# second-state/qwen3_asr_rs

Hardware: NVIDIA H100
Metric: real-time factor (audio-sec/wall-sec) Qwen3-ASR-0.6B 30s clips (higher is better)
Workload: dtype f32 (bf16 weights, fp32-exact activations)

## Files before the change

### qwen3_asr_rs_b200/csrc/decode_batch.cu

```cuda
#include <algorithm>
#include "mega_common.cuh"

namespace asrb {

namespace megab {
using namespace mega;

static constexpr int MAXSPLIT = 32;
static constexpr int MAXROWS = 8;
static constexpr int ATT_SCRATCH = 4 * HD + NCONS_WARPS * 2 * HD + NCONS_WARPS * 4 + 8 + 8 + 2 * HD;

struct Params {
    const DecLayerW* layers;
    const bf16* lm_head;
    const bf16* embed;
    const float* final_norm;
    const float* rope_cos; const float* rope_sin;
    float eps;
    int L, H, QD, KVD, I, V, nkv;
    int nb;
    float* x;
    float* kcache; float* vcache; size_t cache_layer_stride, cache_seq_stride; int max_ctx;
    float* part_val; int* part_idx; int n_part;
    int* pos; int* done; int* next_id; int* ids_out; int* n_out; int max_new;
// ... 46 lines not shown
            const uint32_t xrow = xp + (uint32_t)sq * (H * 2) + (uint32_t)swz16(xc0 + 2 * ks + bhalf, sq & 7) * 16u;
            uint32_t b00, b01, b10, b11, b20, b21;
            ldsm_x4(xrow + (uint32_t)bpl * PSTR, b00, b01, b10, b11);
            ldsm_x2(xrow + 2u * PSTR, b20, b21);
            mma16816(acc[nt], a0, a1, a2, a3, b00, b01);
            mma16816(acc1[nt], a0, a1, a2, a3, b10, b11);
            mma16816(acc2[nt], a0, a1, a2, a3, b20, b21);
        }
    }
#pragma unroll
    for (int nt = 0; nt < NT; ++nt)
#pragma unroll
        for (int k = 0; k < 4; ++k) acc[nt][k] += acc1[nt][k] + acc2[nt][k];
}

static constexpr uint32_t SX_EMPTY = 0xFFFFFFFFu;
__device__ __forceinline__ void sx_store(uint32_t* p, float v) {
    uint32_t b = __float_as_uint(v);
    if (b == SX_EMPTY) b = 0x7FFFFFFFu;
    asm volatile("red.relaxed.gpu.global.and.b32 [%0], %1;" ::"l"(p), "r"(b) : "memory");
}
__device__ __forceinline__ uint4 sx_load4(const uint32_t* p) {
    uint4 v;
    asm volatile("ld.relaxed.gpu.global.v4.u32 {%0, %1, %2, %3}, [%4];" : "=r"(v.x), "=r"(v.y), "=r"(v.z), "=r"(v.w) : "l"(p) : "memory");
    return v;
}

__device__ __forceinline__ void head_norm_rope_b(const uint2* __restrict__ src, uint32_t tag, const float* __restrict__ nw,
                                                 float eps, const float* __restrict__ cs, const float* __restrict__ sn,
                                                 float* dst, int lane) {
    float v[4];
    ll_poll4(src + lane, 32, tag, v);
    const float ss = warp_sum(v[0] * v[0] + v[1] * v[1] + v[2] * v[2] + v[3] * v[3]);
    const float r = 1.0f / sqrtf(ss / 128.f + eps);
#pragma unroll
    for (int i = 0; i < 4; ++i) v[i] = (v[i] * r) * __ldg(nw + lane + 32 * i);
#pragma unroll
    for (int i = 0; i < 2; ++i) {
        const int d = lane + 32 * i;
        const float c = cs[d], s = sn[d];
        const float a = v[i], b = v[i + 2];
// ... 755 lines not shown
```

### qwen3_asr_rs_b200/csrc/decode_mega.cu

```cuda
#include "mega_common.cuh"

namespace asrb {

namespace mega {

struct Params {
    const DecLayerW* layers;
    const bf16* lm_head;
    const bf16* embed;
    const float* final_norm;
    const float* rope_cos; const float* rope_sin;
    float eps;
    int L, H, QD, KVD, I, V, nq, nkv, group;
    float* x;
    float* kcache; float* vcache; size_t cache_layer_stride; int max_ctx;
    int nsplit;
    float* part_val; int* part_idx;
    int* pos; int* done; int* next_id; int* ids_out; int* n_out; int max_new;
    unsigned* bar;
    uint2* qkv_ll; uint2* part_ll; uint2* attn_ll; uint2* x_ll; uint2* act_ll;
    long long* dbg;
};

static_assert(KV_KEYS * HD * 4 == SLOT_BYTES, "K / V tiles travel through the weight ring: one tile per slot");

template <int K>
__device__ __forceinline__ void load_xr(const float* xs, float (&xr)[K / 32], int lane) {
    const int sw = ((lane >> 2) & 1) * 4;
#pragma unroll
    for (int c = 0; c < K / 256; ++c) {
        const float4 a = *reinterpret_cast<const float4*>(xs + (c * 32 + lane) * 8 + sw);
        const float4 b = *reinterpret_cast<const float4*>(xs + (c * 32 + lane) * 8 + 4 - sw);
        xr[c * 8 + 0] = a.x; xr[c * 8 + 1] = a.y; xr[c * 8 + 2] = a.z; xr[c * 8 + 3] = a.w;
        xr[c * 8 + 4] = b.x; xr[c * 8 + 5] = b.y; xr[c * 8 + 6] = b.z; xr[c * 8 + 7] = b.w;
    }
// ... 94 lines not shown
}

__device__ __forceinline__ float warp_reduce8(const float (&a)[8], int lane) {
    const bool h16 = lane & 16, h8 = lane & 8, h4 = lane & 4;
    float k[4];
#pragma unroll
    for (int i = 0; i < 4; ++i) k[i] = (h16 ? a[4 + i] : a[i]) + __shfl_xor_sync(0xffffffffu, h16 ? a[i] : a[4 + i], 16);
    float m0 = (h8 ? k[2] : k[0]) + __shfl_xor_sync(0xffffffffu, h8 ? k[0] : k[2], 8);
    float m1 = (h8 ? k[3] : k[1]) + __shfl_xor_sync(0xffffffffu, h8 ? k[1] : k[3], 8);
    float v = (h4 ? m1 : m0) + __shfl_xor_sync(0xffffffffu, h4 ? m0 : m1, 4);
    v += __shfl_xor_sync(0xffffffffu, v, 2);
    v += __shfl_xor_sync(0xffffffffu, v, 1);
    return v;
}

enum { ME_STORE = 0, ME_RESID = 1, ME_SWIGLU = 2, ME_ARGMAX = 3 };

template <int K>
__device__ __forceinline__ void consume_ksplit(const Slice& s, const Ring& ring, uint32_t& q, const float* xs, uint2* out,
                                               uint32_t tag, float* xres, float* part) {
    const int tid = threadIdx.x, lane = tid & 31, warp = tid >> 5;
    constexpr int NU = K / 8;
    constexpr int J = (NU + NCONS - 1) / NCONS;
    uint32_t grp = 0;
    for (int r = s.r0; r < s.r1;) {
        const int rowsA = min(s.rpc, s.r1 - r);
        const uint32_t slotA = q % ring.nslot;
        mbar_wait(&ring.full[slotA], (q / ring.nslot) & 1);
        const bool pair = s.rpc < 8 && r + rowsA < s.r1;
        const int rowsB = pair ? min(s.rpc, s.r1 - r - rowsA) : 0;
        const uint32_t slotB = (q + 1) % ring.nslot;
        if (pair) mbar_wait(&ring.full[slotB], ((q + 1) / ring.nslot) & 1);
        const uint4* baseA = reinterpret_cast<const uint4*>(ring.slots + (size_t)slotA * SLOT_BYTES);
        const uint4* baseB = reinterpret_cast<const uint4*>(ring.slots + (size_t)slotB * SLOT_BYTES);
        const int R = rowsA + rowsB;
// ... 29 lines not shown
            }
            const float v = warp_reduce8(acc, lane);
            if (g0 + 8 >= R) {
                __syncwarp();
                if (lane == 0) { mbar_arrive(&ring.empty[slotA]); if (pair) mbar_arrive(&ring.empty[slotB]); }
            }
            float* pb = part + (grp & 1) * 64;
            if ((lane & 3) == 0) pb[warp * 8 + (lane >> 2)] = v;
            cons_sync();
            if (tid < ng) {
                float t = pb[tid];
#pragma unroll
                for (int w8 = 1; w8 < NCONS_WARPS; ++w8) t += pb[w8 * 8 + tid];
                const int row = r + g0 + tid;
                const float nv = xres[row - s.r0] + t; xres[row - s.r0] = nv;
                ll_store(out + row, nv, tag);
            }
        }
        r += R; q += pair ? 2 : 1;
    }
}

template <int K, int EPI>
__device__ __forceinline__ void consume_quad(const Slice& s, const Ring& ring, uint32_t& q, const float* xs, uint2* out,
                                             uint32_t tag, float& best_v, int& best_i,
                                             const float* norm_w, float norm_r, long long* fine) {
    const int lane = threadIdx.x & 31, warp = threadIdx.x >> 5;
    int fi = 0;
#define CF() do { if (fine && threadIdx.x == 0 && fi < 24) fine[fi++] = clock64(); } while (0)
    CF();
    constexpr int NU = K / 8;
    float xr[K / 32];
    if (norm_w) load_xr_norm<K>(xs, norm_w, norm_r, xr, lane);
    else load_xr<K>(xs, xr, lane);
    cons_sync();
    CF();
    const int j = lane >> 3;
    for (int r = s.r0; r < s.r1;) {
        const int rowsA = min(s.rpc, s.r1 - r);
        const uint32_t slotA = q % ring.nslot;
// ... 6 lines not shown
        const uint4* baseA = reinterpret_cast<const uint4*>(ring.slots + (size_t)slotA * SLOT_BYTES);
        const uint4* baseB = reinterpret_cast<const uint4*>(ring.slots + (size_t)slotB * SLOT_BYTES);
        const int R = rowsA + rowsB;
        for (int i0 = 4 * warp; i0 < R; i0 += 4 * NCONS_WARPS) {
            const int nv = min(4, R - i0);
            const uint4* rp[4];
#pragma unroll
            for (int i = 0; i < 4; ++i) {
                const int ri = i0 + (i < nv ? i : 0);
                rp[i] = ri < rowsA ? baseA + (size_t)ri * NU : baseB + (size_t)(ri - rowsA) * NU;
            }
            const float v = row_dot4<K>(rp[0], rp[1], rp[2], rp[3], xr, lane);
            const int row = r + i0 + j;
            if (EPI == ME_SWIGLU) {
                const float up = __shfl_xor_sync(0xffffffffu, v, 8);
                if ((lane & 15) == 0 && j < nv) ll_store(out + (row >> 1), silu(v) * up, tag);
            } else if (EPI == ME_STORE) {
                if ((lane & 7) == 0 && j < nv) ll_store(out + row, v, tag);
            } else {
                if ((lane & 7) == 0 && j < nv && v > best_v) { best_v = v; best_i = row; }
            }
        }
        CF();
        __syncwarp();
        if (lane == 0) { mbar_arrive(&ring.empty[slotA]); if (pair) mbar_arrive(&ring.empty[slotB]); }
        r += R; q += pair ? 2 : 1;
    }
    CF();
#undef CF
}

template <int K, int EPI>
__device__ __forceinline__ void consume(const Slice& s, const Ring& ring, uint32_t& q, const float* xs, uint2* out,
                                        uint32_t tag, float* xres, float& best_v, int& best_i,
                                        const float* norm_w = nullptr, float norm_r = 1.f, long long* fine = nullptr,
                                        float* part = nullptr) {
    if constexpr (EPI == ME_RESID) { consume_ksplit<K>(s, ring, q, xs, out, tag, xres, part); return; }
    else if constexpr (K <= 1024) { consume_quad<K, EPI>(s, ring, q, xs, out, tag, best_v, best_i, norm_w, norm_r, fine); return; }
    const int lane = threadIdx.x & 31, warp = threadIdx.x >> 5;
    int fi = 0;
#define CF() do { if (fine && threadIdx.x == 0 && fi < 24) fine[fi++] = clock64(); } while (0)
    CF();
    constexpr int RSTEP = (EPI == ME_SWIGLU) ? 2 : 1;
    constexpr bool XREG = K <= 2048;
    constexpr bool DUAL = XREG && K <= 1024;
    constexpr int KX = XREG ? K : 256;
    constexpr int UPW = (DUAL && EPI != ME_SWIGLU) ? 2 : 1;
    const int sub = lane >> 4;
    float xr[XREG ? K / 32 : 1];
    if (XREG) {
        if (norm_w) load_xr_norm<KX>(xs, norm_w, norm_r, reinterpret_cast<float (&)[KX / 32]>(xr), lane);
        else load_xr<KX>(xs, reinterpret_cast<float (&)[KX / 32]>(xr), lane);
        cons_sync();
// ... 11 lines not shown
        for (int ub = first * UPW; ub < units_here; ub += NCONS_WARPS * UPW) {
            if (EPI == ME_SWIGLU) {
                const int row = r + ub * 2;
                float v0, v1;
                if (DUAL) {
                    const float v = row_dot2<KX>(base + (size_t)(ub * 2) * (K / 8), base + (size_t)(ub * 2 + 1) * (K / 8),
                                                 reinterpret_cast<const float (&)[KX / 32]>(xr), lane);
                    v0 = v; v1 = __shfl_xor_sync(0xffffffffu, v, 16);
                } else if (XREG) {
                    v0 = row_dot<KX>(base + (size_t)(ub * 2) * (K / 8), reinterpret_cast<const float (&)[KX / 32]>(xr), lane);
                    v1 = row_dot<KX>(base + (size_t)(ub * 2 + 1) * (K / 8), reinterpret_cast<const float (&)[KX / 32]>(xr), lane);
                } else {
                    v0 = row_dot_smem<K>(base + (size_t)(ub * 2) * (K / 8), xs, lane);
                    v1 = row_dot_smem<K>(base + (size_t)(ub * 2 + 1) * (K / 8), xs, lane);
                }
                if (lane == 0) ll_store(out + (row >> 1), silu(v0) * v1, tag);
            } else {
                bool act; int row; float v0;
                if (DUAL) {
                    const bool two = ub + 1 < units_here;
                    v0 = row_dot2<KX>(base + (size_t)ub * (K / 8), base + (size_t)(two ? ub + 1 : ub) * (K / 8),
                                      reinterpret_cast<const float (&)[KX / 32]>(xr), lane);
                    act = ((lane & 15) == 0) && (sub == 0 || two);
                    row = r + ub + sub;
                } else {
                    if (XREG) v0 = row_dot<KX>(base + (size_t)ub * (K / 8), reinterpret_cast<const float (&)[KX / 32]>(xr), lane);
                    else v0 = row_dot_smem<K>(base + (size_t)ub * (K / 8), xs, lane);
                    act = lane == 0; row = r + ub;
                }
                if (EPI == ME_STORE) {
                    if (act) ll_store(out + row, v0, tag);
                } else if (EPI == ME_RESID) {
                    if (act) { const float nv = xres[row - s.r0] + v0; xres[row - s.r0] = nv; ll_store(out + row, nv, tag); }
                } else {
                    if (act && v0 > best_v) { best_v = v0; best_i = row; }
                }
            }
        }
        unit += (units_here + UPW - 1) / UPW * UPW;
        CF();
        __syncwarp();
        if (lane == 0) mbar_arrive(&ring.empty[slot]);
    }
    CF();
#undef CF
    if (!XREG) cons_sync();
}

__device__ __forceinline__ float norm_scale(float ss, int n, float eps, float* red) {
    const int tid = threadIdx.x;
    ss = warp_sum(ss);
    if ((tid & 31) == 0) red[tid >> 5] = ss;
    cons_sync();
    float tot = 0.f;
#pragma unroll
    for (int i = 0; i < NCONS_WARPS; ++i) tot += red[i];
    return 1.0f / sqrtf(tot / n + eps);
}

__device__ __forceinline__ void head_norm_rope(const uint2* __restrict__ src, uint32_t tag, const float* __restrict__ nw,
                                               float eps, const float* __restrict__ cs, const float* __restrict__ sn,
// ... 60 lines not shown
        asm volatile("fence.mbarrier_init.release.cluster;" ::: "memory");
    }
    const int pos = __ldcg(p.pos);
    {
        const uint2* src = reinterpret_cast<const uint2*>(p.layers);
        uint2* dst = reinterpret_cast<uint2*>(ltab);
        for (int i = tid; i < p.L * (int)(sizeof(DecLayerW) / 8); i += NTHREADS) dst[i] = src[i];
        if (tid < 64) ropes[tid] = p.rope_cos[(size_t)pos * 64 + tid];
        else if (tid < 128) ropes[tid] = p.rope_sin[(size_t)pos * 64 + tid - 64];
    }
    __syncthreads();

    const bool att_cta = (int)blockIdx.x < p.nkv * p.nsplit;
    const int att_g = blockIdx.x / p.nsplit, att_sp = blockIdx.x % p.nsplit, att_j0 = att_sp * KV_KEYS;
    const int n_old = att_cta ? max(0, min(pos - att_j0, KV_KEYS)) : 0;
    uint32_t q = 0;
    if (is_producer) {
        if (lane == 0) {
            const uint64_t pol = l2_evict_first_policy();
            auto issue = [&](const void* src, uint32_t bytes) __attribute__((always_inline)) {
                const uint32_t slot = q % NS, par = (q / NS) & 1;
                mbar_wait(&ring.empty[slot], par ^ 1);
                mbar_expect_tx(&ring.full[slot], bytes);
                bulk_g2s_hint(ring.slots + (size_t)slot * SLOT_BYTES, src, bytes, &ring.full[slot], pol);
                ++q;
            };
            auto issue_slice = [&](const Slice& s) __attribute__((always_inline)) {
                for (int r = s.r0; r < s.r1; r += s.rpc) issue(s.W + (size_t)r * s.K, (uint32_t)min(s.rpc, s.r1 - r) * s.K * 2);
            };
            const size_t kv_row = ((size_t)att_g * p.max_ctx + att_j0) * HD;
// ... 28 lines not shown
            issue_slice(make_slice(p.lm_head, p.V, H, 1));
        }
        return;
    }

    long long* dbg_row = nullptr; int dbg_i = 0;
    if (p.dbg && (blockIdx.x == 0 || blockIdx.x == gridDim.x - 1)) dbg_row = p.dbg + (blockIdx.x == 0 ? 0 : DBG_SLOTS);
    MEGA_MARK();
    const int half = HD / 2;
    const float* cs = ropes;
    const float* sn = ropes + half;
    const unsigned G = gridDim.x;
    float best_v = -INFINITY; int best_i = 0x7fffffff;
    const unsigned epoch = __ldcg(p.bar + 1);
    const uint32_t tag_base = (epoch & 0xffffffu) << 8;
    const Slice xsl = make_slice(nullptr, H, QD, 1);
    Slice sl_qkv = make_slice(nullptr, QD + 2 * p.KVD, H, 1), sl_o = make_slice(nullptr, H, QD, 1),
          sl_gu = make_slice(nullptr, 2 * I, H, 2), sl_dn = make_slice(nullptr, H, I, 1);
    for (int i = tid; i < xsl.r1 - xsl.r0; i += NCONS) xres[i] = __ldcg(p.x + xsl.r0 + i);

    for (int l = 0; l < p.L; ++l) {
        const DecLayerW w = ltab[l];
        const uint32_t tl = tag_base | ((uint32_t)l << 3);
        const float* pb = pbuf + (l & 1) * PARAM_FLOATS;
        mbar_wait(&p_full[l & 1], (l >> 1) & 1);
        float nr;
        {
            float ss = 0.f;
            if (l == 0) { for (int i = tid; i < H; i += NCONS) { const float v = __ldcg(p.x + i); xs[xs_swz(i)] = v; ss = fmaf(v, v, ss); } }
            else { MEGA_FINE(0); MEGA_FINE(1); ss = ll_gather(p.x_ll, H, (tag_base | ((uint32_t)(l - 1) << 3)) | PH_XD, xs); MEGA_FINE(2); }
            nr = norm_scale(ss, H, p.eps, red);
            MEGA_FINE(3);
        }
        consume<H, ME_STORE>(sl_qkv, ring, q, xs, p.qkv_ll, tl | PH_QKV, xres, best_v, best_i, pb, nr);
        MEGA_FINE(4);
        MEGA_GT(0);
        MEGA_MARK();
        {
            const int nloc = n_old;
            const int nact = min(p.nsplit, (pos + KV_KEYS - 1) / KV_KEYS);
            const bool merger = att_cta && att_sp == 0;
            if (nloc > 0) {
                const int g = att_g;
                float* qs = xs;
                float* kn = qs + p.group * HD;
                float* vn = kn + HD;
                float* sc = vn + HD;
                float* ml = sc + p.group * KV_KEYS;
                float* osum = ml + 8;
                float* wml = osum + NCONS_WARPS * 2 * HD;
                float* snew = wml + NCONS_WARPS * 4;
                const uint32_t ksl = q % ring.nslot, vsl = (q + 1) % ring.nslot;
                const float* Ks = reinterpret_cast<const float*>(ring.slots + (size_t)ksl * SLOT_BYTES);
                const float* Vs = reinterpret_cast<const float*>(ring.slots + (size_t)vsl * SLOT_BYTES);
                MEGA_FINE(24);
                cons_sync();
// ... 169 lines not shown
                            ok = __all_sync(0xffffffffu, (mv.y == tg) && (lv.y == tg) && round_ok(0));
                        } while (!ok);
                        MEGA_FINE(35);
                        const float m_l = lane < nact ? __uint_as_float(mv.x) : (lane == nact ? snew[hq] : -INFINITY);
                        const float l_l = lane < nact ? __uint_as_float(lv.x) : (lane == nact ? 1.f : 0.f);
                        const float M = warp_max(m_l);
                        const float f = expf(m_l - M);
                        const float Lsum = warp_sum(f * l_l);
                        float O = __shfl_sync(0xffffffffu, f, nact) * vn[d];
                        for (int u0 = 0; u0 < nact; u0 += RB) {
                            if (u0 > 0) { do { load_round(u0); ok = __all_sync(0xffffffffu, round_ok(u0)); } while (!ok); }
#pragma unroll
                            for (int u = 0; u < RB; ++u)
                                if (u0 + u < nact) O = fmaf(__shfl_sync(0xffffffffu, f, u0 + u), __uint_as_float(ov[u].x), O);
                        }
                        ll_store(p.attn_ll + (size_t)(g * p.group + hq) * HD + d, O / Lsum, tl | PH_ATTN);
                    }
                }
                MEGA_FINE(31);
                cons_sync();
            }
        }
        MEGA_MARK();
        MEGA_FINE(32);
        ll_gather(p.attn_ll, QD, tl | PH_ATTN, xs);
        MEGA_FINE(33);
        MEGA_GT(2);
        cons_sync();
        consume<QD, ME_RESID>(sl_o, ring, q, xs, p.x_ll, tl | PH_XO, xres, best_v, best_i, nullptr, 1.f, nullptr, part);
        MEGA_FINE(34);
        MEGA_MARK();
        cons_sync();
        {
            MEGA_FINE(8); MEGA_FINE(9);
            const float ss = ll_gather(p.x_ll, H, tl | PH_XO, xs); MEGA_FINE(10);
            nr = norm_scale(ss, H, p.eps, red); MEGA_FINE(11);
        }
        consume<H, ME_SWIGLU>(sl_gu, ring, q, xs, p.act_ll, tl | PH_ACT, xres, best_v, best_i, pb + H, nr, (dbg_row && l == 5) ? dbg_row + 440 : nullptr);
        MEGA_FINE(12);
        MEGA_FINE(13);
        MEGA_MARK();
        MEGA_FINE(16); MEGA_FINE(17);
        ll_gather(p.act_ll, I, tl | PH_ACT, xs); MEGA_FINE(18);
        cons_sync();
        consume<I, ME_RESID>(sl_dn, ring, q, xs, p.x_ll, tl | PH_XD, xres, best_v, best_i, nullptr, 1.f, nullptr, part);
        MEGA_FINE(19);
        MEGA_FINE(20);
        MEGA_MARK();
        cons_sync();
        if (lane == 0) mbar_arrive(&p_empty[l & 1]);
    }
    float nrf;
    {
        const float ss = ll_gather(p.x_ll, H, (tag_base | ((uint32_t)(p.L - 1) << 3)) | PH_XD, xs);
        mbar_wait(&p_full[p.L & 1], (p.L >> 1) & 1);
        nrf = norm_scale(ss, H, p.eps, red);
    }
    consume<H, ME_ARGMAX>(make_slice(p.lm_head, p.V, H, 1), ring, q, xs, nullptr, 0u, xres, best_v, best_i,
                          pbuf + (p.L & 1) * PARAM_FLOATS, nrf);
    MEGA_MARK();
#pragma unroll
    for (int o = 8; o <= 16; o <<= 1) {
        const float ov = __shfl_xor_sync(0xffffffffu, best_v, o); const int oi = __shfl_xor_sync(0xffffffffu, best_i, o);
        if (ov > best_v || (ov == best_v && oi < best_i)) { best_v = ov; best_i = oi; }
    }
    cons_sync();
    if (lane == 0) { red[warp] = best_v; ired[warp] = best_i; }
    cons_sync();
    int& is_last = ired[63];
    if (tid == 0) {
        float v = -INFINITY; int idx = 0x7fffffff;
        for (int wq = 0; wq < NCONS_WARPS; ++wq)
            if (red[wq] > v || (red[wq] == v && ired[wq] < idx)) { v = red[wq]; idx = ired[wq]; }
// ... 17 lines not shown
            if (ov > v || (ov == v && oi < idx)) { v = ov; idx = oi; }
        }
        if (lane == 0) { red[warp] = v; ired[warp] = idx; }
        cons_sync();
        int& tok_s = ired[62];
        if (tid == 0) {
            for (int wq = 1; wq < NCONS_WARPS; ++wq)
                if (red[wq] > v || (red[wq] == v && ired[wq] < idx)) { v = red[wq]; idx = ired[wq]; }
            int tok = idx;
            const int n = *p.n_out;
            if (tok == 151643 || tok == 151645 || n >= p.max_new) { *p.done = 1; *p.next_id = -1; tok = -1; }
            else { p.ids_out[n] = tok; *p.n_out = n + 1; *p.pos = pos + 1; *p.next_id = tok; }
            tok_s = tok;
            p.bar[0] = 0;
            p.bar[1] = p.bar[1] + 1;
        }
        cons_sync();
        const int tok = tok_s;
        if (tok >= 0) {
            const bf16* e = p.embed + (size_t)tok * H;
            for (int i = tid; i < H; i += NCONS) p.x[i] = __bfloat162float(e[i]);
        }
    }
}

}

static long long* g_last_dbg = nullptr;

static int mega_xs_floats(int I) { return std::max(I, mega::XS_MIN) + 64; }
// ... 14 lines not shown
    if (B < 1 || c.head_dim != 128) return false;
    const int group = c.num_attention_heads / c.num_key_value_heads;
    if (group + 2 > mega::NCONS_WARPS) return false;
    if ((size_t)(group * 128 + 256 + group * mega::KV_KEYS + 8 + mega::NCONS_WARPS * 2 * 128 + mega::NCONS_WARPS * 4 + 8) > (size_t)mega_xs_floats(c.intermediate_size)) return false;
    if (m.ctx->smem_optin < mega_smem_bytes(c.hidden_size, c.intermediate_size, mega_nslot(c))) return false;
    if ((c.hidden_size + m.ctx->sm_count - 1) / m.ctx->sm_count + 1 > mega::XRES_MAX) return false;
    if (c.num_hidden_layers > 32) return false;
    if ((max_ctx + mega::KV_KEYS - 1) / mega::KV_KEYS > mega::MAX_SPLITS) return false;
    if (((max_ctx + mega::KV_KEYS - 1) / mega::KV_KEYS) * c.num_key_value_heads > m.ctx->sm_count) return false;
    return dims_match<1024, 2048, 3072>(c) || dims_match<2048, 2048, 6144>(c) || dims_match<256, 512, 512>(c);
}

size_t decode_mega_part_floats(const Model& m) {
    const asrb_dims& c = m.d.c;
    const int group = c.num_attention_heads / c.num_key_value_heads;
    const size_t words = (size_t)m.d.qkv_dim + (size_t)m.ctx->sm_count * group * mega::PSTRIDE + m.d.q_dim + c.hidden_size +
                         c.intermediate_size + 64;
    return 2 * words + 64;
}

void launch_decode_step_mega(const Model& m, const DecodeBufs& b, int B, float* kcache, float* vcache,
                             size_t cache_layer_stride, size_t cache_seq_stride, int max_ctx, int ctx_now, const MegaBufs& mb,
                             cudaStream_t st, int64_t* launches) {
    ASRB_REQUIRE(decode_mega_supported(m, B, ctx_now), ASRB_ERR_STATE, "fused decode step not supported for this model/batch/context");
    ASRB_REQUIRE(m.d_dec_layers && mb.bar && mb.part, ASRB_ERR_STATE, "fused decode step buffers missing");
    const asrb_dims& c = m.d.c;
    const int G = m.ctx->sm_count;
    const int group = c.num_attention_heads / c.num_key_value_heads;
    const int nsplit = std::min(mega::MAX_SPLITS, std::min(G / c.num_key_value_heads, (max_ctx + mega::KV_KEYS - 1) / mega::KV_KEYS));
    const size_t smem = mega_smem_bytes(c.hidden_size, c.intermediate_size, mega_nslot(c));
    const void* fn = nullptr;
    if (dims_match<1024, 2048, 3072>(c)) fn = (const void*)mega::decode_step_kernel<1024, 2048, 3072, 6>;
    else if (dims_match<2048, 2048, 6144>(c)) fn = (const void*)mega::decode_step_kernel<2048, 2048, 6144, 5>;
    else fn = (const void*)mega::decode_step_kernel<256, 512, 512, 6>;
    ASRB_CUDA_CHECK(cudaFuncSetAttribute(fn, cudaFuncAttributeMaxDynamicSharedMemorySize, (int)smem));
    for (int sb = 0; sb < B; ++sb) {
        mega::Params p{};
        p.layers = m.d_dec_layers; p.lm_head = m.lm_head; p.embed = m.embed; p.final_norm = m.final_norm_sw;
        p.rope_cos = m.rope_cos; p.rope_sin = m.rope_sin; p.eps = (float)c.rms_norm_eps;
        p.L = c.num_hidden_layers; p.H = c.hidden_size; p.QD = m.d.q_dim; p.KVD = m.d.kv_dim; p.I = c.intermediate_size;
        p.V = c.vocab_size; p.nq = c.num_attention_heads; p.nkv = c.num_key_value_heads; p.group = group;
        p.x = b.x + (size_t)sb * c.hidden_size;
        p.kcache = kcache + (size_t)sb * cache_seq_stride; p.vcache = vcache + (size_t)sb * cache_seq_stride;
        p.cache_layer_stride = cache_layer_stride; p.max_ctx = max_ctx; p.nsplit = nsplit;
        p.part_val = b.part_val; p.part_idx = b.part_idx;
        p.pos = b.pos + sb; p.done = b.done + sb; p.next_id = b.next_id + sb;
        p.ids_out = b.ids_out + (size_t)sb * b.max_new; p.n_out = b.n_out + sb; p.max_new = b.max_new;
        p.bar = mb.bar;
        uint2* w = reinterpret_cast<uint2*>(mb.part);
        p.qkv_ll = w; w += m.d.qkv_dim;
        p.part_ll = w; w += (size_t)G * group * mega::PSTRIDE;
        p.attn_ll = w; w += m.d.q_dim;
        p.x_ll = w; w += c.hidden_size;
        p.act_ll = w; w += c.intermediate_size;
        p.dbg = mb.dbg;
        g_last_dbg = mb.dbg;
        if (mb.steps_issued && ++*mb.steps_issued >= 0xFFFF00u) {
            ASRB_CUDA_CHECK(cudaMemsetAsync(mb.part, 0, mb.part_bytes, st));
            const unsigned one = 1;
            ASRB_CUDA_CHECK(cudaMemcpyAsync(mb.bar + 1, &one, sizeof(one), cudaMemcpyHostToDevice, st));
            *mb.steps_issued = 1;
        }
        void* args[] = {(void*)&p};
        ASRB_CUDA_CHECK(cudaLaunchCooperativeKernel(fn, dim3(G), dim3(mega::NTHREADS), args, smem, st));
        if (launches) *launches += 1;
    }
}

int decode_mega_debug_timeline(long long* out, int cap) {
// ... 9 lines not shown
```

### qwen3_asr_rs_b200/csrc/internal.h

```cpp
#pragma once
#include <atomic>
#include <map>
#include <string>
#include <vector>
#include "../../include/asr_b200.h"
#include "common.cuh"

namespace asrb {

struct Dims {
    asrb_dims c;
    int enc_hd;
    int chunk_frames;
    int chunks_per_window;
    int conv_h[4];
    int conv_w[4];
    int tok_per_chunk;
    int cpad;
    int feat;
    int q_dim, kv_dim, qkv_dim;
    void derive();
};
void validate_dims(const asrb_dims& d);
inline int conv_out_len(int l) { return (l - 1) / 2 + 1; }
// ... 121 lines not shown
    float* attn;
    float* act;
    float* logits;
    float* part_val; int* part_idx; int n_part;
    int* pos;
    int* done;
    int* next_id;
    int* ids_out;
    int* n_out;
    int max_new;
};
void launch_decode_step_phases(const Model& m, const DecodeBufs& b, int B, float* kcache, float* vcache,
                               size_t cache_layer_stride, size_t cache_seq_stride, int max_ctx,
                               bool write_logits, cudaStream_t st, int64_t* launches);
struct MegaBufs { unsigned* bar = nullptr; float* part = nullptr; long long* dbg = nullptr; size_t part_bytes = 0; unsigned* steps_issued = nullptr;
                  uint32_t* sx = nullptr; size_t sx_bytes = 0; int* sx_nb = nullptr; };
size_t decode_mega_part_floats(const Model& m);
size_t decode_batch_part_floats(const Model& m);
size_t decode_batch_sx_bytes(const Model& m);
bool decode_batch_supported(const Model& m, int B, int ctx);
int decode_mega_dbg_slots();
void launch_greedy(const Model& m, const DecodeBufs& b, int B, cudaStream_t st, int64_t* launches);
void launch_lmhead_argmax(const Model& m, const float* x_rows, const int* d_row_idx, int B,
                          const DecodeBufs& b, bool write_logits, cudaStream_t st, int64_t* launches);

}
```

### qwen3_asr_rs_b200/csrc/mega_common.cuh

```cuda
#pragma once
#include "internal.h"

namespace asrb {
namespace mega {

static constexpr int NCONS_WARPS = 8;
static constexpr int NCONS = NCONS_WARPS * 32;
static constexpr int NTHREADS = NCONS + 32;
static constexpr int SLOT_BYTES = 32 * 1024;
static constexpr int NSLOT_MAX = 6;
static constexpr int KV_KEYS = 64;
static constexpr int XS_MIN = 3072;
static constexpr int XRES_MAX = 64;
static constexpr int MAX_LAYERS = 32;
static constexpr int HD = 128;
static constexpr int PSTRIDE = HD + 2;
static constexpr int DBG_SLOTS = 1024;
static constexpr int MAX_SPLITS = 18;

enum { PH_QKV = 1, PH_PART = 2, PH_ATTN = 3, PH_XO = 4, PH_ACT = 5, PH_XD = 6 };

__device__ __forceinline__ uint32_t smem_u32(const void* p) { return (uint32_t)__cvta_generic_to_shared(p); }
__device__ __forceinline__ void mbar_init(uint64_t* bar, uint32_t count) {
    asm volatile("mbarrier.init.shared::cta.b64 [%0], %1;" ::"r"(smem_u32(bar)), "r"(count));
}
__device__ __forceinline__ void mbar_expect_tx(uint64_t* bar, uint32_t bytes) {
    asm volatile("mbarrier.arrive.expect_tx.shared::cta.b64 _, [%0], %1;" ::"r"(smem_u32(bar)), "r"(bytes) : "memory");
}
__device__ __forceinline__ void mbar_arrive(uint64_t* bar) {
    asm volatile("mbarrier.arrive.shared::cta.b64 _, [%0];" ::"r"(smem_u32(bar)) : "memory");
}
__device__ __forceinline__ void mbar_wait(uint64_t* bar, uint32_t parity) {
    asm volatile(
        "{\n"
        ".reg .pred p;\n"
// ... 11 lines not shown
__device__ __forceinline__ uint64_t l2_evict_first_policy() {
    uint64_t pol;
    asm volatile("createpolicy.fractional.L2::evict_first.b64 %0, 1.0;" : "=l"(pol));
    return pol;
}
__device__ __forceinline__ void bulk_g2s_hint(void* dst, const void* src, uint32_t bytes, uint64_t* bar, uint64_t pol) {
    asm volatile("cp.async.bulk.shared::cluster.global.mbarrier::complete_tx::bytes.L2::cache_hint [%0], [%1], %2, [%3], %4;"
                 ::"r"(smem_u32(dst)), "l"(src), "r"(bytes), "r"(smem_u32(bar)), "l"(pol) : "memory");
}
__device__ __forceinline__ void cons_sync() { asm volatile("bar.sync 1, %0;" ::"n"(NCONS) : "memory"); }

__device__ __forceinline__ void ll_store(uint2* p, float v, uint32_t tag) {
    const unsigned long long val = ((unsigned long long)tag << 32) | (unsigned long long)__float_as_uint(v);
    asm volatile("red.relaxed.gpu.global.max.u64 [%0], %1;" ::"l"(p), "l"(val) : "memory");
}
__device__ __forceinline__ uint4 ll_load2(const uint2* p) {
    uint4 v;
    asm volatile("ld.relaxed.gpu.global.v4.u32 {%0, %1, %2, %3}, [%4];" : "=r"(v.x), "=r"(v.y), "=r"(v.z), "=r"(v.w) : "l"(p) : "memory");
    return v;
}
__device__ __forceinline__ float ll_poll1(const uint2* p, uint32_t tag) {
    uint2 v;
    do {
        asm volatile("ld.relaxed.gpu.global.v2.u32 {%0, %1}, [%2];" : "=r"(v.x), "=r"(v.y) : "l"(p) : "memory");
    } while (v.y != tag);
    return __uint_as_float(v.x);
}
__device__ __forceinline__ void ll_poll4(const uint2* p, int stride, uint32_t tag, float (&out)[4]) {
    uint2 v[4];
    bool ok;
    do {
#pragma unroll
        for (int i = 0; i < 4; ++i)
            asm volatile("ld.relaxed.gpu.global.v2.u32 {%0, %1}, [%2];" : "=r"(v[i].x), "=r"(v[i].y) : "l"(p + (size_t)i * stride) : "memory");
        ok = (v[0].y == tag) && (v[1].y == tag) && (v[2].y == tag) && (v[3].y == tag);
    } while (!ok);
#pragma unroll
    for (int i = 0; i < 4; ++i) out[i] = __uint_as_float(v[i].x);
}
__device__ __forceinline__ int xs_swz(int e) { const int k = e >> 2; return ((k ^ ((k >> 3) & 1)) << 2) | (e & 3); }
__device__ __forceinline__ float ll_gather(const uint2* buf, int n, uint32_t tag, float* xs) {
    float ss = 0.f;
    const int pairs = n >> 1;
    constexpr int U = 8;
    for (int i0 = threadIdx.x; i0 < pairs; i0 += U * NCONS) {
        uint4 v[U];
#pragma unroll
        for (int u = 0; u < U; ++u) v[u] = make_uint4(0u, 0u, 0u, 0u);
        bool ok;
        do {
            ok = true;
#pragma unroll
            for (int u = 0; u < U; ++u) {
                const int i = i0 + u * NCONS;
                if (i < pairs && !(v[u].y == tag && v[u].w == tag)) v[u] = ll_load2(buf + 2 * i);
            }
#pragma unroll
            for (int u = 0; u < U; ++u) {
                const int i = i0 + u * NCONS;
                if (i < pairs) ok = ok && (v[u].y == tag) && (v[u].w == tag);
            }
        } while (!ok);
#pragma unroll
        for (int u = 0; u < U; ++u) {
            const int i = i0 + u * NCONS;
            if (i < pairs) {
                const float a = __uint_as_float(v[u].x), b = __uint_as_float(v[u].z);
                *reinterpret_cast<float2*>(xs + xs_swz(2 * i)) = make_float2(a, b);
                ss = fmaf(a, a, ss); ss = fmaf(b, b, ss);
            }
        }
    }
    return ss;
}

struct Ring {
    uint8_t* slots; uint64_t* full; uint64_t* empty;
    uint32_t nslot;
};

struct Slice { const bf16* W; int K, r0, r1, rpc; };
__device__ __forceinline__ Slice make_slice(const bf16* W, int N, int K, int rstep) {
    Slice s; s.W = W; s.K = K;
    const unsigned units = (unsigned)(N / rstep);
    const int u0 = (int)((blockIdx.x * units) / gridDim.x), u1 = (int)(((blockIdx.x + 1) * units) / gridDim.x);
    s.r0 = u0 * rstep; s.r1 = u1 * rstep;
    s.rpc = SLOT_BYTES / (K * 2);
    s.rpc &= ~1;
    return s;
// ... 5 lines not shown
```

### qwen3_asr_rs_b200/csrc/session.cu

```cuda
#include <algorithm>
#include <cstring>
#include "internal.h"

namespace asrb {

void model_set_tensor(Model* m, const char* name, int dtype, const int64_t* shape, int ndim, const void* host);
void model_finalize(Model* m);
struct IngestState;
IngestState* ingest_state_new();
void ingest_state_free(IngestState* st);
void ingest_pcm(IngestState* st, cudaStream_t stream, const void* const* pcm, const int64_t* n_frames, const int32_t* channels,
                const int32_t* rate, const int32_t* format, int batch, float* d_samples, int64_t max_samples_per_utt,
                int64_t* n_out, int64_t* soff_out);

static const int kPromptHead[9] = {151644, 8948, 198, 151645, 198, 151644, 872, 198, 151669};
static const int kPromptTail[6] = {151670, 151645, 198, 151644, 77091, 198};
static const int kAudioPad = 151676;

struct Session {
    Model* m = nullptr;
    cudaStream_t st = nullptr;
    int max_batch = 0, max_lang = 0, max_new = 0;
    int64_t max_samples = 0, max_npad = 0;
    int maxF = 0, maxC = 0, maxT = 0, maxS = 0, max_ctx = 0;
// ... 145 lines not shown
            s->mega.sx_nb = &s->sx_nb;
            int maxwin = 0, maxpersist = 0;
            cudaDeviceGetAttribute(&maxwin, cudaDevAttrMaxAccessPolicyWindowSize, m->ctx->device);
            cudaDeviceGetAttribute(&maxpersist, cudaDevAttrMaxPersistingL2CacheSize, m->ctx->device);
            if (maxwin > 0 && maxpersist > 0) {
                const size_t want = std::min<size_t>({s->mega.sx_bytes, (size_t)maxwin, (size_t)maxpersist});
                if (cudaDeviceSetLimit(cudaLimitPersistingL2CacheSize, want) == cudaSuccess) {
                    cudaStreamAttrValue av{};
                    av.accessPolicyWindow.base_ptr = s->mega.sx; av.accessPolicyWindow.num_bytes = want;
                    av.accessPolicyWindow.hitRatio = 1.0f; av.accessPolicyWindow.hitProp = cudaAccessPropertyPersisting;
                    av.accessPolicyWindow.missProp = cudaAccessPropertyStreaming;
                    if (cudaStreamSetAttribute(s->st, cudaStreamAttributeAccessPolicyWindow, &av) != cudaSuccess) cudaGetLastError();
                } else cudaGetLastError();
            }
        }
        if (getenv("ASRB_MEGA_DEBUG")) s->mega.dbg = salloc<long long>(s, decode_mega_dbg_slots(), true);
        ASRB_CUDA_CHECK(cudaMallocHost(&s->h_done, Bm * sizeof(int)));
        ASRB_CUDA_CHECK(cudaMallocHost(&s->h_nout, Bm * sizeof(int)));
        ASRB_CUDA_CHECK(cudaMallocHost(&s->h_next, Bm * sizeof(int)));
        ASRB_CUDA_CHECK(cudaMallocHost(&s->h_ids, Bm * max_new * sizeof(int)));
        ASRB_CUDA_CHECK(cudaDeviceSynchronize());
    } catch (...) { delete s; throw; }
    return s;
}

void session_free(Session* s) { delete s; }

void session_mel(Session* s, const float* const* samples, const int64_t* n_samples, int batch, int64_t* n_frames_out) {
    ASRB_REQUIRE(batch >= 1 && batch <= s->max_batch, ASRB_ERR_INVALID, "batch exceeds session capacity");
    ASRB_CUDA_CHECK(cudaSetDevice(s->m->ctx->device));
// ... 410 lines not shown
```

Before: 292.9.

## Replace tagged LL exchange buffers with double-buffered sentinel slots in mega decode

The single-sequence megakernel now exchanges the residual, attention output and MLP activation between CTAs through per-layer, per-step double-buffered 32-bit slots. These slots are pre-filled with an all-ones sentinel and written with an atomic AND, replacing the 64-bit tagged LL stores. Readers poll 16-byte vectors until no word is empty, which halves the exchanged bytes and drops the tag compares. Each CTA re-arms its slice of the other parity buffer at step start, and a new step counter selects the parity. This adds re-arming work and a memory footprint of 2×L layer buffers.

Measured after the change: 301.9, median of 6. +3.1%, better.

```diff
diff --git a/qwen3_asr_rs_b200/csrc/decode_batch.cu b/qwen3_asr_rs_b200/csrc/decode_batch.cu
--- a/qwen3_asr_rs_b200/csrc/decode_batch.cu
+++ b/qwen3_asr_rs_b200/csrc/decode_batch.cu
@@ -84,17 +84,6 @@
         for (int k = 0; k < 4; ++k) acc[nt][k] += acc1[nt][k] + acc2[nt][k];
 }
 
-static constexpr uint32_t SX_EMPTY = 0xFFFFFFFFu;
-__device__ __forceinline__ void sx_store(uint32_t* p, float v) {
-    uint32_t b = __float_as_uint(v);
-    if (b == SX_EMPTY) b = 0x7FFFFFFFu;
-    asm volatile("red.relaxed.gpu.global.and.b32 [%0], %1;" ::"l"(p), "r"(b) : "memory");
-}
-__device__ __forceinline__ uint4 sx_load4(const uint32_t* p) {
-    uint4 v;
-    asm volatile("ld.relaxed.gpu.global.v4.u32 {%0, %1, %2, %3}, [%4];" : "=r"(v.x), "=r"(v.y), "=r"(v.z), "=r"(v.w) : "l"(p) : "memory");
-    return v;
-}
 
 __device__ __forceinline__ void head_norm_rope_b(const uint2* __restrict__ src, uint32_t tag, const float* __restrict__ nw,
                                                  float eps, const float* __restrict__ cs, const float* __restrict__ sn,
diff --git a/qwen3_asr_rs_b200/csrc/decode_mega.cu b/qwen3_asr_rs_b200/csrc/decode_mega.cu
--- a/qwen3_asr_rs_b200/csrc/decode_mega.cu
+++ b/qwen3_asr_rs_b200/csrc/decode_mega.cu
@@ -18,7 +18,8 @@
     float* part_val; int* part_idx;
     int* pos; int* done; int* next_id; int* ids_out; int* n_out; int max_new;
     unsigned* bar;
-    uint2* qkv_ll; uint2* part_ll; uint2* attn_ll; uint2* x_ll; uint2* act_ll;
+    uint2* qkv_ll; uint2* part_ll;
+    uint32_t* sx;
     long long* dbg;
 };
 
@@ -143,11 +144,11 @@
     return v;
 }
 
-enum { ME_STORE = 0, ME_RESID = 1, ME_SWIGLU = 2, ME_ARGMAX = 3 };
+enum { ME_STORE = 0, ME_SWIGLU = 1, ME_ARGMAX = 2 };
 
 template <int K>
-__device__ __forceinline__ void consume_ksplit(const Slice& s, const Ring& ring, uint32_t& q, const float* xs, uint2* out,
-                                               uint32_t tag, float* xres, float* part) {
+__device__ __forceinline__ void consume_ksplit(const Slice& s, const Ring& ring, uint32_t& q, const float* xs, uint32_t* out,
+                                               float* xres, float* part) {
     const int tid = threadIdx.x, lane = tid & 31, warp = tid >> 5;
     constexpr int NU = K / 8;
     constexpr int J = (NU + NCONS - 1) / NCONS;
@@ -207,7 +208,7 @@
                 for (int w8 = 1; w8 < NCONS_WARPS; ++w8) t += pb[w8 * 8 + tid];
                 const int row = r + g0 + tid;
                 const float nv = xres[row - s.r0] + t; xres[row - s.r0] = nv;
-                ll_store(out + row, nv, tag);
+                sx_store(out + row, nv);
             }
         }
         r += R; q += pair ? 2 : 1;
@@ -216,7 +217,7 @@
 
 template <int K, int EPI>
 __device__ __forceinline__ void consume_quad(const Slice& s, const Ring& ring, uint32_t& q, const float* xs, uint2* out,
-                                             uint32_t tag, float& best_v, int& best_i,
+                                             uint32_t tag, uint32_t* sxo, float& best_v, int& best_i,
                                              const float* norm_w, float norm_r, long long* fine) {
     const int lane = threadIdx.x & 31, warp = threadIdx.x >> 5;
     int fi = 0;
@@ -253,7 +254,7 @@
             const int row = r + i0 + j;
             if (EPI == ME_SWIGLU) {
                 const float up = __shfl_xor_sync(0xffffffffu, v, 8);
-                if ((lane & 15) == 0 && j < nv) ll_store(out + (row >> 1), silu(v) * up, tag);
+                if ((lane & 15) == 0 && j < nv) sx_store(sxo + (row >> 1), silu(v) * up);
             } else if (EPI == ME_STORE) {
                 if ((lane & 7) == 0 && j < nv) ll_store(out + row, v, tag);
             } else {
@@ -271,11 +272,9 @@
 
 template <int K, int EPI>
 __device__ __forceinline__ void consume(const Slice& s, const Ring& ring, uint32_t& q, const float* xs, uint2* out,
-                                        uint32_t tag, float* xres, float& best_v, int& best_i,
-                                        const float* norm_w = nullptr, float norm_r = 1.f, long long* fine = nullptr,
-                                        float* part = nullptr) {
-    if constexpr (EPI == ME_RESID) { consume_ksplit<K>(s, ring, q, xs, out, tag, xres, part); return; }
-    else if constexpr (K <= 1024) { consume_quad<K, EPI>(s, ring, q, xs, out, tag, best_v, best_i, norm_w, norm_r, fine); return; }
+                                        uint32_t tag, uint32_t* sxo, float& best_v, int& best_i,
+                                        const float* norm_w = nullptr, float norm_r = 1.f, long long* fine = nullptr) {
+    if constexpr (K <= 1024) { consume_quad<K, EPI>(s, ring, q, xs, out, tag, sxo, best_v, best_i, norm_w, norm_r, fine); return; }
     const int lane = threadIdx.x & 31, warp = threadIdx.x >> 5;
     int fi = 0;
 #define CF() do { if (fine && threadIdx.x == 0 && fi < 24) fine[fi++] = clock64(); } while (0)
@@ -317,7 +316,7 @@
                     v0 = row_dot_smem<K>(base + (size_t)(ub * 2) * (K / 8), xs, lane);
                     v1 = row_dot_smem<K>(base + (size_t)(ub * 2 + 1) * (K / 8), xs, lane);
                 }
-                if (lane == 0) ll_store(out + (row >> 1), silu(v0) * v1, tag);
+                if (lane == 0) sx_store(sxo + (row >> 1), silu(v0) * v1);
             } else {
                 bool act; int row; float v0;
                 if (DUAL) {
@@ -333,8 +332,6 @@
                 }
                 if (EPI == ME_STORE) {
                     if (act) ll_store(out + row, v0, tag);
-                } else if (EPI == ME_RESID) {
-                    if (act) { const float nv = xres[row - s.r0] + v0; xres[row - s.r0] = nv; ll_store(out + row, nv, tag); }
                 } else {
                     if (act && v0 > best_v) { best_v = v0; best_i = row; }
                 }
@@ -348,6 +345,50 @@
     CF();
 #undef CF
     if (!XREG) cons_sync();
+}
+
+template <int N>
+__device__ __forceinline__ float sx_gather(const uint32_t* src, float* xs) {
+    const int tid = threadIdx.x, lane = tid & 31, warp = tid >> 5;
+    constexpr int NQ = N / 4;
+    constexpr int KQ = (NQ + NCONS - 1) / NCONS;
+    int qi[KQ];
+    uint4 v[KQ];
+#pragma unroll
+    for (int k = 0; k < KQ; ++k) {
+        qi[k] = 16 * warp + (lane & 15) + (NCONS / 2) * (2 * k + (lane >> 4));
+        v[k] = make_uint4(SX_EMPTY, SX_EMPTY, SX_EMPTY, SX_EMPTY);
+    }
+    bool ok;
+    do {
+        ok = true;
+#pragma unroll
+        for (int k = 0; k < KQ; ++k)
+            if (qi[k] < NQ && !sx_ready(v[k])) v[k] = sx_load4(src + 4 * qi[k]);
+#pragma unroll
+        for (int k = 0; k < KQ; ++k)
+            if (qi[k] < NQ) ok = ok && sx_ready(v[k]);
+    } while (!ok);
+#pragma unroll
+    for (int k = 0; k < KQ; ++k)
+        if (qi[k] < NQ) *reinterpret_cast<uint4*>(xs + xs_swz(4 * qi[k])) = v[k];
+    __syncwarp();
+    float ss = 0.f;
+#pragma unroll
+    for (int i = tid; i < N / 2; i += NCONS) {
+        const float2 x = *reinterpret_cast<const float2*>(xs + xs_swz(2 * i));
+        ss = fmaf(x.x, x.x, ss); ss = fmaf(x.y, x.y, ss);
+    }
+    return ss;
+}
+
+template <int N>
+__device__ __forceinline__ void sx_copy(const uint32_t* src, float* xs) {
+    for (int j = threadIdx.x; j < N / 4; j += NCONS) {
+        uint4 v;
+        do { v = sx_load4(src + 4 * j); } while (!sx_ready(v));
+        *reinterpret_cast<uint4*>(xs + xs_swz(4 * j)) = v;
+    }
 }
 
 __device__ __forceinline__ float norm_scale(float ss, int n, float eps, float* red) {
@@ -438,6 +479,20 @@
     const bool att_cta = (int)blockIdx.x < p.nkv * p.nsplit;
     const int att_g = blockIdx.x / p.nsplit, att_sp = blockIdx.x % p.nsplit, att_j0 = att_sp * KV_KEYS;
     const int n_old = att_cta ? max(0, min(pos - att_j0, KV_KEYS)) : 0;
+    const bool merger = att_cta && att_sp == 0;
+    const Slice xsl = make_slice(nullptr, H, QD, 1), sl_gu = make_slice(nullptr, 2 * I, H, 2);
+
+    constexpr size_t SXL = 2 * H + QD + I;
+    const unsigned sstep = __ldcg(p.bar + 3);
+    uint32_t* const sx_cur = p.sx + (size_t)(sstep & 1u) * p.L * SXL;
+    auto rearm = [&](int l) __attribute__((always_inline)) {
+        uint32_t* const base = p.sx + (size_t)((sstep & 1u) ^ 1u) * p.L * SXL + (size_t)l * SXL;
+        const int xrows = xsl.r1 - xsl.r0, a0 = sl_gu.r0 / 2, arows = sl_gu.r1 / 2 - a0;
+        const int nattn = merger ? p.group * HD : 0;
+        for (int i = tid; i < xrows; i += NCONS) { base[xsl.r0 + i] = SX_EMPTY; base[H + xsl.r0 + i] = SX_EMPTY; }
+        for (int i = tid; i < nattn; i += NCONS) base[2 * H + att_g * p.group * HD + i] = SX_EMPTY;
+        for (int i = tid; i < arows; i += NCONS) base[2 * H + QD + a0 + i] = SX_EMPTY;
+    };
     uint32_t q = 0;
     if (is_producer) {
         if (lane == 0) {
@@ -496,32 +551,34 @@
     float best_v = -INFINITY; int best_i = 0x7fffffff;
     const unsigned epoch = __ldcg(p.bar + 1);
     const uint32_t tag_base = (epoch & 0xffffffu) << 8;
-    const Slice xsl = make_slice(nullptr, H, QD, 1);
-    Slice sl_qkv = make_slice(nullptr, QD + 2 * p.KVD, H, 1), sl_o = make_slice(nullptr, H, QD, 1),
-          sl_gu = make_slice(nullptr, 2 * I, H, 2), sl_dn = make_slice(nullptr, H, I, 1);
+    Slice sl_qkv = make_slice(nullptr, QD + 2 * p.KVD, H, 1), sl_o = make_slice(nullptr, H, QD, 1), sl_dn = make_slice(nullptr, H, I, 1);
     for (int i = tid; i < xsl.r1 - xsl.r0; i += NCONS) xres[i] = __ldcg(p.x + xsl.r0 + i);
+    for (int l = 0; l < p.L; ++l) rearm(l);
 
     for (int l = 0; l < p.L; ++l) {
         const DecLayerW w = ltab[l];
         const uint32_t tl = tag_base | ((uint32_t)l << 3);
         const float* pb = pbuf + (l & 1) * PARAM_FLOATS;
+        uint32_t* const sx_xo = sx_cur + (size_t)l * SXL;
+        uint32_t* const sx_xd = sx_xo + H;
+        uint32_t* const sx_attn = sx_xo + 2 * H;
+        uint32_t* const sx_act = sx_xo + 2 * H + QD;
         mbar_wait(&p_full[l & 1], (l >> 1) & 1);
         float nr;
         {
             float ss = 0.f;
             if (l == 0) { for (int i = tid; i < H; i += NCONS) { const float v = __ldcg(p.x + i); xs[xs_swz(i)] = v; ss = fmaf(v, v, ss); } }
-            else { MEGA_FINE(0); MEGA_FINE(1); ss = ll_gather(p.x_ll, H, (tag_base | ((uint32_t)(l - 1) << 3)) | PH_XD, xs); MEGA_FINE(2); }
+            else { MEGA_FINE(0); MEGA_FINE(1); ss = sx_gather<H>(sx_xd - SXL, xs); MEGA_FINE(2); }
             nr = norm_scale(ss, H, p.eps, red);
             MEGA_FINE(3);
         }
-        consume<H, ME_STORE>(sl_qkv, ring, q, xs, p.qkv_ll, tl | PH_QKV, xres, best_v, best_i, pb, nr);
+        consume<H, ME_STORE>(sl_qkv, ring, q, xs, p.qkv_ll, tl | PH_QKV, nullptr, best_v, best_i, pb, nr);
         MEGA_FINE(4);
         MEGA_GT(0);
         MEGA_MARK();
         {
             const int nloc = n_old;
             const int nact = min(p.nsplit, (pos + KV_KEYS - 1) / KV_KEYS);
-            const bool merger = att_cta && att_sp == 0;
             if (nloc > 0) {
                 const int g = att_g;
                 float* qs = xs;
@@ -721,7 +778,7 @@
                             for (int u = 0; u < RB; ++u)
                                 if (u0 + u < nact) O = fmaf(__shfl_sync(0xffffffffu, f, u0 + u), __uint_as_float(ov[u].x), O);
                         }
-                        ll_store(p.attn_ll + (size_t)(g * p.group + hq) * HD + d, O / Lsum, tl | PH_ATTN);
+                        sx_store(sx_attn + (size_t)(g * p.group + hq) * HD + d, O / Lsum);
                     }
                 }
                 MEGA_FINE(31);
@@ -730,27 +787,27 @@
         }
         MEGA_MARK();
         MEGA_FINE(32);
-        ll_gather(p.attn_ll, QD, tl | PH_ATTN, xs);
+        sx_copy<QD>(sx_attn, xs);
         MEGA_FINE(33);
         MEGA_GT(2);
         cons_sync();
-        consume<QD, ME_RESID>(sl_o, ring, q, xs, p.x_ll, tl | PH_XO, xres, best_v, best_i, nullptr, 1.f, nullptr, part);
+        consume_ksplit<QD>(sl_o, ring, q, xs, sx_xo, xres, part);
         MEGA_FINE(34);
         MEGA_MARK();
         cons_sync();
         {
             MEGA_FINE(8); MEGA_FINE(9);
-            const float ss = ll_gather(p.x_ll, H, tl | PH_XO, xs); MEGA_FINE(10);
+            const float ss = sx_gather<H>(sx_xo, xs); MEGA_FINE(10);
             nr = norm_scale(ss, H, p.eps, red); MEGA_FINE(11);
         }
-        consume<H, ME_SWIGLU>(sl_gu, ring, q, xs, p.act_ll, tl | PH_ACT, xres, best_v, best_i, pb + H, nr, (dbg_row && l == 5) ? dbg_row + 440 : nullptr);
+        consume<H, ME_SWIGLU>(sl_gu, ring, q, xs, nullptr, 0u, sx_act, best_v, best_i, pb + H, nr, (dbg_row && l == 5) ? dbg_row + 440 : nullptr);
         MEGA_FINE(12);
         MEGA_FINE(13);
         MEGA_MARK();
         MEGA_FINE(16); MEGA_FINE(17);
-        ll_gather(p.act_ll, I, tl | PH_ACT, xs); MEGA_FINE(18);
+        sx_copy<I>(sx_act, xs); MEGA_FINE(18);
         cons_sync();
-        consume<I, ME_RESID>(sl_dn, ring, q, xs, p.x_ll, tl | PH_XD, xres, best_v, best_i, nullptr, 1.f, nullptr, part);
+        consume_ksplit<I>(sl_dn, ring, q, xs, sx_xd, xres, part);
         MEGA_FINE(19);
         MEGA_FINE(20);
         MEGA_MARK();
@@ -759,11 +816,11 @@
     }
     float nrf;
     {
-        const float ss = ll_gather(p.x_ll, H, (tag_base | ((uint32_t)(p.L - 1) << 3)) | PH_XD, xs);
+        const float ss = sx_gather<H>(sx_cur + (size_t)(p.L - 1) * SXL + H, xs);
         mbar_wait(&p_full[p.L & 1], (p.L >> 1) & 1);
         nrf = norm_scale(ss, H, p.eps, red);
     }
-    consume<H, ME_ARGMAX>(make_slice(p.lm_head, p.V, H, 1), ring, q, xs, nullptr, 0u, xres, best_v, best_i,
+    consume<H, ME_ARGMAX>(make_slice(p.lm_head, p.V, H, 1), ring, q, xs, nullptr, 0u, nullptr, best_v, best_i,
                           pbuf + (p.L & 1) * PARAM_FLOATS, nrf);
     MEGA_MARK();
 #pragma unroll
@@ -811,6 +868,7 @@
             tok_s = tok;
             p.bar[0] = 0;
             p.bar[1] = p.bar[1] + 1;
+            p.bar[3] = p.bar[3] + 1;
         }
         cons_sync();
         const int tok = tok_s;
@@ -855,16 +913,19 @@
 size_t decode_mega_part_floats(const Model& m) {
     const asrb_dims& c = m.d.c;
     const int group = c.num_attention_heads / c.num_key_value_heads;
-    const size_t words = (size_t)m.d.qkv_dim + (size_t)m.ctx->sm_count * group * mega::PSTRIDE + m.d.q_dim + c.hidden_size +
-                         c.intermediate_size + 64;
+    const size_t words = (size_t)m.d.qkv_dim + (size_t)m.ctx->sm_count * group * mega::PSTRIDE + 64;
     return 2 * words + 64;
+}
+size_t decode_mega_sx_bytes(const Model& m) {
+    const asrb_dims& c = m.d.c;
+    return 2 * (size_t)c.num_hidden_layers * (2 * (size_t)c.hidden_size + m.d.q_dim + c.intermediate_size) * sizeof(uint32_t);
 }
 
 void launch_decode_step_mega(const Model& m, const DecodeBufs& b, int B, float* kcache, float* vcache,
                              size_t cache_layer_stride, size_t cache_seq_stride, int max_ctx, int ctx_now, const MegaBufs& mb,
                              cudaStream_t st, int64_t* launches) {
     ASRB_REQUIRE(decode_mega_supported(m, B, ctx_now), ASRB_ERR_STATE, "fused decode step not supported for this model/batch/context");
-    ASRB_REQUIRE(m.d_dec_layers && mb.bar && mb.part, ASRB_ERR_STATE, "fused decode step buffers missing");
+    ASRB_REQUIRE(m.d_dec_layers && mb.bar && mb.part && mb.sx_seq, ASRB_ERR_STATE, "fused decode step buffers missing");
     const asrb_dims& c = m.d.c;
     const int G = m.ctx->sm_count;
     const int group = c.num_attention_heads / c.num_key_value_heads;
@@ -890,10 +951,8 @@
         p.bar = mb.bar;
         uint2* w = reinterpret_cast<uint2*>(mb.part);
         p.qkv_ll = w; w += m.d.qkv_dim;
-        p.part_ll = w; w += (size_t)G * group * mega::PSTRIDE;
-        p.attn_ll = w; w += m.d.q_dim;
-        p.x_ll = w; w += c.hidden_size;
-        p.act_ll = w; w += c.intermediate_size;
+        p.part_ll = w;
+        p.sx = mb.sx_seq;
         p.dbg = mb.dbg;
         g_last_dbg = mb.dbg;
         if (mb.steps_issued && ++*mb.steps_issued >= 0xFFFF00u) {
diff --git a/qwen3_asr_rs_b200/csrc/internal.h b/qwen3_asr_rs_b200/csrc/internal.h
--- a/qwen3_asr_rs_b200/csrc/internal.h
+++ b/qwen3_asr_rs_b200/csrc/internal.h
@@ -159,8 +159,10 @@
                                size_t cache_layer_stride, size_t cache_seq_stride, int max_ctx,
                                bool write_logits, cudaStream_t st, int64_t* launches);
 struct MegaBufs { unsigned* bar = nullptr; float* part = nullptr; long long* dbg = nullptr; size_t part_bytes = 0; unsigned* steps_issued = nullptr;
-                  uint32_t* sx = nullptr; size_t sx_bytes = 0; int* sx_nb = nullptr; };
+                  uint32_t* sx = nullptr; size_t sx_bytes = 0; int* sx_nb = nullptr;
+                  uint32_t* sx_seq = nullptr; };
 size_t decode_mega_part_floats(const Model& m);
+size_t decode_mega_sx_bytes(const Model& m);
 size_t decode_batch_part_floats(const Model& m);
 size_t decode_batch_sx_bytes(const Model& m);
 bool decode_batch_supported(const Model& m, int B, int ctx);
diff --git a/qwen3_asr_rs_b200/csrc/mega_common.cuh b/qwen3_asr_rs_b200/csrc/mega_common.cuh
--- a/qwen3_asr_rs_b200/csrc/mega_common.cuh
+++ b/qwen3_asr_rs_b200/csrc/mega_common.cuh
@@ -18,7 +18,7 @@
 static constexpr int DBG_SLOTS = 1024;
 static constexpr int MAX_SPLITS = 18;
 
-enum { PH_QKV = 1, PH_PART = 2, PH_ATTN = 3, PH_XO = 4, PH_ACT = 5, PH_XD = 6 };
+enum { PH_QKV = 1, PH_PART = 2 };
 
 __device__ __forceinline__ uint32_t smem_u32(const void* p) { return (uint32_t)__cvta_generic_to_shared(p); }
 __device__ __forceinline__ void mbar_init(uint64_t* bar, uint32_t count) {
@@ -60,11 +60,6 @@
     const unsigned long long val = ((unsigned long long)tag << 32) | (unsigned long long)__float_as_uint(v);
     asm volatile("red.relaxed.gpu.global.max.u64 [%0], %1;" ::"l"(p), "l"(val) : "memory");
 }
-__device__ __forceinline__ uint4 ll_load2(const uint2* p) {
-    uint4 v;
-    asm volatile("ld.relaxed.gpu.global.v4.u32 {%0, %1, %2, %3}, [%4];" : "=r"(v.x), "=r"(v.y), "=r"(v.z), "=r"(v.w) : "l"(p) : "memory");
-    return v;
-}
 __device__ __forceinline__ float ll_poll1(const uint2* p, uint32_t tag) {
     uint2 v;
     do {
@@ -84,41 +79,22 @@
 #pragma unroll
     for (int i = 0; i < 4; ++i) out[i] = __uint_as_float(v[i].x);
 }
+static constexpr uint32_t SX_EMPTY = 0xFFFFFFFFu;
+__device__ __forceinline__ void sx_store(uint32_t* p, float v) {
+    uint32_t b = __float_as_uint(v);
+    if (b == SX_EMPTY) b = 0x7FFFFFFFu;
+    asm volatile("red.relaxed.gpu.global.and.b32 [%0], %1;" ::"l"(p), "r"(b) : "memory");
+}
+__device__ __forceinline__ uint4 sx_load4(const uint32_t* p) {
+    uint4 v;
+    asm volatile("ld.relaxed.gpu.global.v4.u32 {%0, %1, %2, %3}, [%4];" : "=r"(v.x), "=r"(v.y), "=r"(v.z), "=r"(v.w) : "l"(p) : "memory");
+    return v;
+}
+__device__ __forceinline__ bool sx_ready(const uint4& v) {
+    return v.x != SX_EMPTY && v.y != SX_EMPTY && v.z != SX_EMPTY && v.w != SX_EMPTY;
+}
+
 __device__ __forceinline__ int xs_swz(int e) { const int k = e >> 2; return ((k ^ ((k >> 3) & 1)) << 2) | (e & 3); }
-__device__ __forceinline__ float ll_gather(const uint2* buf, int n, uint32_t tag, float* xs) {
-    float ss = 0.f;
-    const int pairs = n >> 1;
-    constexpr int U = 8;
-    for (int i0 = threadIdx.x; i0 < pairs; i0 += U * NCONS) {
-        uint4 v[U];
-#pragma unroll
-        for (int u = 0; u < U; ++u) v[u] = make_uint4(0u, 0u, 0u, 0u);
-        bool ok;
-        do {
-            ok = true;
-#pragma unroll
-            for (int u = 0; u < U; ++u) {
-                const int i = i0 + u * NCONS;
-                if (i < pairs && !(v[u].y == tag && v[u].w == tag)) v[u] = ll_load2(buf + 2 * i);
-            }
-#pragma unroll
-            for (int u = 0; u < U; ++u) {
-                const int i = i0 + u * NCONS;
-                if (i < pairs) ok = ok && (v[u].y == tag) && (v[u].w == tag);
-            }
-        } while (!ok);
-#pragma unroll
-        for (int u = 0; u < U; ++u) {
-            const int i = i0 + u * NCONS;
-            if (i < pairs) {
-                const float a = __uint_as_float(v[u].x), b = __uint_as_float(v[u].z);
-                *reinterpret_cast<float2*>(xs + xs_swz(2 * i)) = make_float2(a, b);
-                ss = fmaf(a, a, ss); ss = fmaf(b, b, ss);
-            }
-        }
-    }
-    return ss;
-}
 
 struct Ring {
     uint8_t* slots; uint64_t* full; uint64_t* empty;
diff --git a/qwen3_asr_rs_b200/csrc/session.cu b/qwen3_asr_rs_b200/csrc/session.cu
--- a/qwen3_asr_rs_b200/csrc/session.cu
+++ b/qwen3_asr_rs_b200/csrc/session.cu
@@ -183,6 +183,11 @@
                 } else cudaGetLastError();
             }
         }
+        {
+            const size_t bytes = decode_mega_sx_bytes(*m);
+            s->mega.sx_seq = (uint32_t*)salloc<uint8_t>(s, bytes);
+            ASRB_CUDA_CHECK(cudaMemset(s->mega.sx_seq, 0xFF, bytes));
+        }
         if (getenv("ASRB_MEGA_DEBUG")) s->mega.dbg = salloc<long long>(s, decode_mega_dbg_slots(), true);
         ASRB_CUDA_CHECK(cudaMallocHost(&s->h_done, Bm * sizeof(int)));
         ASRB_CUDA_CHECK(cudaMallocHost(&s->h_nout, Bm * sizeof(int)));
```
